# astaka-pe/Dual-DMP

Measured on AMD Instinct MI355X. Metric: training iters/sec + MAD score, 1M-face mesh @ 1/2/4/8 MI355X, higher is better.
Workload: dtype f32 (f16x3 split-MFMA GEMMs, f32 accumulate); 1 GPU; synthetic torus-grid manifold mesh, 1000000 faces / 500000 verts, float32 features, k=(3,4,4,4,1), bnfloop=1, native numbering (BASELINE.json configs[2]); faces=1000000, verts=500000, parallelism=1 GPU, hipgraph_replay=True, two_streams=True

## Files before the change

### dual-dmp_amd/csrc/gemm.hip

```cpp
#include "ddmp_common.h"
#include "finalize.h"
#include "gemm_tn_rm.h"

#include <algorithm>
#include <cstdlib>
#include <type_traits>
#include <vector>

namespace {

using namespace ddmp;

typedef float f32x16 __attribute__((ext_vector_type(16)));

constexpr int kBM = 128;
constexpr int kBK = 32;
constexpr int kLd = kBK + 4;

template <int TN, bool B_KMAJOR, bool PRO>
__global__ __launch_bounds__(256) void gemm_rows_kernel(
    const float* __restrict__ A, int64_t lda, const float* __restrict__ B, int64_t ldb,
    float* __restrict__ Y, int64_t ldy, int n_rows, int KD, int MD,
    const float* __restrict__ bias, const float* __restrict__ pscale, const float* __restrict__ pshift,
    float slope, int n_row_tiles, int n_col_tiles) {
// ... 471 lines not shown
                            int64_t n_rows) {
    return panel_enabled() && n_rows >= panel_min_rows(KD, MD) && KD % 32 == 0 && KD >= 32 && (KD >= 64 || MD <= 128) &&
           MD % 4 == 0 && MD >= 16 && MD <= 512 && ws &&
           (reinterpret_cast<uintptr_t>(ws) & 15) == 0 && ws_bytes >= ddmp_gemm_rows_workspace_bytes(KD, MD) &&
           ldy >= MD && Y;
}
static bool rr_enabled() {
    static int e = -1;
    if (e < 0) {
        const char* v = getenv("DDMP_GEMM_RR");
        e = (v && atoi(v) == 0) ? 0 : 1;
    }
    return e == 1;
}
static inline bool rr_route_ok(int64_t n_rows, int KD, int64_t lda, int64_t lda2) {
    return rr_enabled() && KD >= 64 && KD <= 512 && n_rows >= kRRMinRows &&
           n_rows * lda * 4 < ((int64_t)1 << 32) && n_rows * lda2 * 4 < ((int64_t)1 << 32);
}
template <int PM>
static void f16s_measure(const float* A, int64_t lda, const float* A2, int64_t lda2, int64_t n_rows, int C,
                         const float* pa, const float* pb, const float* pk1, const float* pk0, float slope, float* slot,
                         hipStream_t st) {
    (void)hipMemsetAsync(slot, 0, 16, st);
    const int64_t total = n_rows * (C / 4);
    const int grid = (int)std::min<int64_t>(cdiv(total, 256 * 8), 8 * device_cus());
    hipLaunchKernelGGL((f16s_absmax_kernel<PM>), dim3((unsigned)std::max(grid, 1)), dim3(256), 0, st, A, lda, A2, lda2,
                       n_rows, C, pa, pb, pk1, pk0, slope, slot);
}

template <int PM>
static void launch_panel(int mode, const float* A, int64_t lda, const float* A2, int64_t lda2, const float* W,
                         int64_t ldw, int transpose, void* planes, float* Y, int64_t ldy, int n_rows, int KD, int MD,
                         const float* bias, const float* ps, const float* psh, const float* pc1, const float* pc0,
                         float slope, hipStream_t st, double* stats, double* sums, ddmp::CallCtx& ctx,
                         const float* red_yp = nullptr, int64_t red_ldyp = 0,
                         const float* const* red_bn4 = nullptr ) {
    const int WC = MD > 256 ? 4 : MD > 128 ? 2 : 1, WR = 8 / WC;
    const int NJ = MD > 128 ? 4 : MD > 64 ? 4 : MD > 32 ? 2 : 1;
    const int MP = 32 * NJ * WC, BMR = 64 * WR;
    const int n_row_tiles = (int)ddmp::cdiv(n_rows, BMR);
    const int64_t total = (int64_t)MP * KD;
    const int sgrid = (int)std::min<int64_t>(ddmp::cdiv(total, 256), 1024);
    dim3 grid((unsigned)std::min(n_row_tiles, device_cus())), block(512);
    const int f16 = (mode == 6 && WC > 1 && lda % 4 == 0 && (PM != 2 || lda2 % 4 == 0)) ? gemm_f16() : 0;
    if (f16) {
        char* tail = (char*)planes + (size_t)2 * MP * KD * 2;
        float* wscale = (float*)tail;
        float* slot = ctx.slot_a ? ctx.slot_a : (float*)(tail + 16);
        const bool prime = !ctx.slot_a || ctx.prime;
        const bool w_ready = w_prepared(ctx.prepared, W, ldw, planes, kWPanelF16, 2, MD, KD, transpose, MP);
        if (!w_ready) {
            (void)hipMemsetAsync(wscale, 0, 4, st);
            hipLaunchKernelGGL(f16s_wmax_kernel, dim3((unsigned)std::min(transpose ? KD : MD, 128)), dim3(256), 0, st, W, ldw,
                               transpose ? KD : MD, transpose ? MD : KD, wscale);
        }
        const bool rr = rr_route_ok(n_rows, KD, lda, PM == 2 ? lda2 : 0) && !(PM == 2 && MD > kRRCols);
        if (!w_ready)
            hipLaunchKernelGGL((split_w_panel_kernel<2, _Float16>), dim3(sgrid), dim3(256), 0, st, W, ldw, MD, KD, transpose, MP,
                               (_Float16*)planes, (const float*)wscale);
        if (prime) f16s_measure<PM>(A, lda, A2, lda2, n_rows, KD, ps, psh, pc1, pc0, slope, slot, st);
        const int target = prime ? kF16TargetExact : kF16TargetStale;
        const void* Bh = planes;
        if (rr) {
            const int n_halves = MP / kRRCols;
            const int tiles = (int)ddmp::cdiv(n_rows, kRRRows);
            const int slots = std::max(8, std::min((tiles + 7) / 8 * 8, 2 * device_cus() / n_halves / 8 * 8));
            dim3 rgrid((unsigned)(slots * n_halves)), rblock(256);
            for (int heal = 0; heal <= (prime ? 0 : 1); ++heal) {
                if (PM == 0 && stats && red_yp)
                    hipLaunchKernelGGL((gemm_rr_kernel<0, 2, 3>), rgrid, rblock, 0, st, A, lda, A2, lda2, (const _Float16*)Bh, MP,
                                       Y, ldy, n_rows, KD, MD, bias, ps, psh, pc1, pc0, slope, tiles, stats, slot,
                                       (const float*)wscale, target, heal, red_yp, red_ldyp, red_bn4[0], red_bn4[1], red_bn4[2],
                                       red_bn4[3]);
                else if (PM != 2 && stats)
                    hipLaunchKernelGGL((gemm_rr_kernel<PM == 2 ? 0 : PM, 1, 3>), rgrid, rblock, 0, st, A, lda, A2, lda2,
                                       (const _Float16*)Bh, MP, Y, ldy, n_rows, KD, MD, bias, ps, psh, pc1, pc0, slope, tiles,
                                       stats, slot, (const float*)wscale, target, heal);
                else
                    hipLaunchKernelGGL((gemm_rr_kernel<PM, 0, PM == 2 ? 2 : 3>), rgrid, rblock, 0, st, A, lda, A2, lda2, (const _Float16*)Bh, MP,
                                       Y, ldy, n_rows, KD, MD, bias, ps, psh, pc1, pc0, slope, tiles, stats, slot,
                                       (const float*)wscale, target, heal);
            }
            if (stats && sums) {
                const size_t pbytes = ((size_t)tiles * 2 * 2 * MP * sizeof(double) + 255) / 256 * 256;
                fpartials_reduce(stats, tiles * 2, MP, MD, (double*)((char*)stats + pbytes), sums, st, ctx.take_fin(MD));
            }
            return;
        }
#define DDMP_PANEL_H(WR_, WC_, AR_, HEAL_)                                                                        \
    hipLaunchKernelGGL((gemm_panel_kernel<WR_, WC_, AR_, PM, 4>), grid, block, 0, st, A, lda, A2, lda2, Bh, Y, ldy,   \
                       n_rows, KD, MD, bias, ps, psh, pc1, pc0, slope, n_row_tiles, stats, slot, (const float*)wscale, \
                       target, HEAL_)
        for (int heal = 0; heal <= (prime ? 0 : 1); ++heal) {
            if (WC == 4) {
                DDMP_PANEL_H(2, 4, 13, heal);
            } else {
                DDMP_PANEL_H(4, 2, 13, heal);
            }
        }
#undef DDMP_PANEL_H
        if (stats && sums) {
            const size_t pbytes = ((size_t)n_row_tiles * WR * 2 * MP * sizeof(double) + 255) / 256 * 256;
            fpartials_reduce(stats, n_row_tiles * WR, MP, MD, (double*)((char*)stats + pbytes), sums, st, ctx.take_fin(MD));
        }
        return;
    }
    if (w_prepared(ctx.prepared, W, ldw, planes, kWPanelB16, mode == 6 ? 3 : 2, MD, KD, transpose, MP)) {
    } else if (mode == 6)
        hipLaunchKernelGGL((split_w_panel_kernel<3, __bf16>), dim3(sgrid), dim3(256), 0, st, W, ldw, MD, KD, transpose, MP, (__bf16*)planes, (const float*)nullptr);
    else
        hipLaunchKernelGGL((split_w_panel_kernel<2, __bf16>), dim3(sgrid), dim3(256), 0, st, W, ldw, MD, KD, transpose, MP, (__bf16*)planes, (const float*)nullptr);
    const void* Bp = planes;
#define DDMP_PANEL(WR_, WC_, NT_, NJ_)                                                                            \
    hipLaunchKernelGGL((gemm_panel_kernel<WR_, WC_, NT_, PM, NJ_>), grid, block, 0, st, A, lda, A2, lda2, Bp, Y, ldy, \
                       n_rows, KD, MD, bias, ps, psh, pc1, pc0, slope, n_row_tiles, stats, (float*)nullptr,            \
                       (const float*)nullptr, 0, 0)
    if (WC == 1 && PM == 0 && stats && red_yp && (NJ == 4 || NJ == 2)) {
#define DDMP_PANEL_RS(NT_, NJ_)                                                                                     \
    hipLaunchKernelGGL((gemm_panel_kernel<8, 1, NT_, 0, NJ_, true>), grid, block, 0, st, A, lda, A2, lda2, Bp, Y, ldy, \
                       n_rows, KD, MD, bias, ps, psh, pc1, pc0, slope, n_row_tiles, stats, (float*)nullptr,            \
                       (const float*)nullptr, 0, 0, red_yp, red_ldyp, red_bn4[0], red_bn4[1], red_bn4[2], red_bn4[3])
        if constexpr (PM == 0) {
            if (NJ == 4) {
                if (mode == 6) DDMP_PANEL_RS(3, 4); else DDMP_PANEL_RS(2, 4);
            } else {
                if (mode == 6) DDMP_PANEL_RS(3, 2); else DDMP_PANEL_RS(2, 2);
            }
        }
#undef DDMP_PANEL_RS
    } else if (WC == 4) {
        if (mode == 6) DDMP_PANEL(2, 4, 3, 4); else DDMP_PANEL(2, 4, 2, 4);
    } else if (WC == 2) {
        if (mode == 6) DDMP_PANEL(4, 2, 3, 4); else DDMP_PANEL(4, 2, 2, 4);
    } else {
        if (NJ == 4) {
            if (mode == 6) DDMP_PANEL(8, 1, 3, 4); else DDMP_PANEL(8, 1, 2, 4);
        } else if (NJ == 2) {
            if (mode == 6) DDMP_PANEL(8, 1, 3, 2); else DDMP_PANEL(8, 1, 2, 2);
        } else {
            if (mode == 6) DDMP_PANEL(8, 1, 3, 1); else DDMP_PANEL(8, 1, 2, 1);
        }
    }
#undef DDMP_PANEL
    if (stats && sums) {
        const size_t pbytes = ((size_t)n_row_tiles * WR * 2 * MP * sizeof(double) + 255) / 256 * 256;
        fpartials_reduce(stats, n_row_tiles * WR, MP, MD, (double*)((char*)stats + pbytes), sums, st, ctx.take_fin(MD));
    }
}

static inline bool ws_ok(int KD, int MD, const float* Y, int64_t ldy, const void* ws, size_t ws_bytes) {
    return ws_enabled() && KD % 32 == 0 && KD >= 96 && MD % 4 == 0 && MD <= 1024 && ldy % 4 == 0 &&
           (reinterpret_cast<uintptr_t>(Y) & 15) == 0 && ws && (reinterpret_cast<uintptr_t>(ws) & 15) == 0 &&
           ws_bytes >= ddmp_gemm_rows_workspace_bytes(KD, MD);
}

static int g_gemm_mode = -1, g_gemm_f16 = 0;
static int gemm_mode() {
    if (g_gemm_mode < 0) {
        const char* e = getenv("DDMP_GEMM_MODE");
        int m = e ? atoi(e) : 13;
        g_gemm_f16 = m == 13 ? m : 0;
        g_gemm_mode = (m == 0 || m == 3 || m == 6) ? m : 6;
    }
    return g_gemm_mode;
}
static int gemm_f16() {
    (void)gemm_mode();
    return g_gemm_f16;
}
extern "C" int ddmp_set_gemm_mode(int mode) {
    if (mode != 0 && mode != 3 && mode != 6 && mode != 13) return DDMP_EINVAL;
    g_gemm_f16 = mode > 10 ? mode : 0;
    g_gemm_mode = mode > 10 ? 6 : mode;
    return DDMP_OK;
}
extern "C" int ddmp_get_gemm_mode(void) { return gemm_f16() ? gemm_f16() : gemm_mode(); }

extern "C" int ddmp_gemm_scales_roll(float* slots, int n_slots, ddmp_stream stream) {
    ARG_TRY(slots && n_slots > 0);
    hipLaunchKernelGGL(f16s_roll_kernel, dim3((unsigned)cdiv(n_slots, 64)), dim3(64), 0, (hipStream_t)stream, slots, n_slots);
    LAUNCH_TRY();
    return DDMP_OK;
}

static inline bool aligned16(const void* p) { return (reinterpret_cast<uintptr_t>(p) & 15) == 0; }

extern "C" size_t ddmp_gemm_rows_workspace_bytes(int K, int M) {
    if (K <= 0 || M <= 0) return 0;
    const size_t kp = ((size_t)K + 127) / 128 * 128, mp = ((size_t)M + 127) / 128 * 128;
    return 3 * kp * mp * 2;
}

static bool presplit_w(const float* W, int64_t ldw, int M, int K, int transpose, void* ws, size_t ws_bytes,
                       hipStream_t st, bool prepared) {
    const int mode = gemm_mode();
    const int RK = transpose ? M : K;
    if (mode == 0 || !ws || ws_bytes < ddmp_gemm_rows_workspace_bytes(K, M) || RK % 8 != 0 ||
        (reinterpret_cast<uintptr_t>(ws) & 15))
        return false;
    const int grid = (int)std::min<int64_t>(cdiv((int64_t)M * K, 256), 1024);
    if (w_prepared(prepared, W, ldw, ws, kWPlain, mode == 6 ? 3 : 2, M, K, transpose, 0)) return true;
    if (mode == 6)
        hipLaunchKernelGGL((split_w_kernel<3>), dim3(grid), dim3(256), 0, st, W, ldw, M, K, transpose, (__bf16*)ws);
    else
        hipLaunchKernelGGL((split_w_kernel<2>), dim3(grid), dim3(256), 0, st, W, ldw, M, K, transpose, (__bf16*)ws);
    return hipGetLastError() == hipSuccess;
}

static WPrepDesc plan_w(int form, int64_t n_rows, const float* W, int64_t ldw, int M, int K, int has_pro, void* planes,
                        size_t planes_bytes) {
    WPrepDesc d{W, planes, ldw, 0, 0, 0, 0, 0, 0};
    const int mode = gemm_mode();
    if (mode == 0 || !planes || (reinterpret_cast<uintptr_t>(planes) & 15) || planes_bytes < ddmp_gemm_rows_workspace_bytes(K, M))
        return d;
    const int KD = form ? M : K, MD = form ? K : M;
    d.transpose = form ? 1 : 0;
    d.nterm = mode == 6 ? 3 : 2;
    float dummy;
    if (!(has_pro && KD > 512) && panel_ok(KD, MD, &dummy, MD, planes, planes_bytes, n_rows)) {
        const int WC = MD > 256 ? 4 : MD > 128 ? 2 : 1;
        const int NJ = MD > 128 ? 4 : MD > 64 ? 4 : MD > 32 ? 2 : 1;
        d.P = 32 * NJ * WC;
        d.MD = MD;
        d.KD = KD;
        if (mode == 6 && WC > 1 && gemm_f16()) {
            d.kind = kWPanelF16;
            d.nterm = 2;
        } else {
            d.kind = kWPanelB16;
// ... 479 lines not shown
```

### dual-dmp_amd/csrc/gemm_panel.inc

```

constexpr int kPanelThreads = 512;

__device__ __forceinline__ int panel_sw(int r, int h) { return r * 16 + ((h ^ ((r >> 3) & 1)) << 3); }

template <int ARITH> struct Arith {
    static constexpr bool F16 = ARITH > 10;
    static constexpr int NTERM = ARITH == 3 ? 3 : 2;
    static constexpr int NP = ARITH == 3 ? 6 : ARITH == 14 ? 4 : 3;
    typedef typename std::conditional<F16, _Float16, __bf16>::type E;
    static constexpr int pa(int q) { return ARITH == 3 ? (q == 0 ? 0 : q == 1 ? 1 : q == 2 ? 2 : q == 3 ? 0 : q == 4 ? 1 : 0)
                                                       : (q == 0 ? 0 : q == 1 ? 1 : NP == 4 && q == 2 ? 1 : 0); }
    static constexpr int pb(int q) { return ARITH == 3 ? (q == 0 ? 2 : q == 1 ? 1 : q == 2 ? 0 : q == 3 ? 1 : 0)
                                                       : (q == 0 ? 1 : q == 1 ? 0 : NP == 4 && q == 2 ? 1 : 0); }
};

#include "gemm_f16s.inc"

template <int NTERM, typename E>
__device__ __forceinline__ void split_w_panel_body(const float* __restrict__ W, int64_t ldw, int MD, int KD, int transpose,
                                                   int MP, E* __restrict__ planes, float ws, int bid, int nblk) {
    const int ns = KD / kSK;
    const int total = ns * MP * kSK;
    for (int idx = bid * 256 + threadIdx.x; idx < total; idx += nblk * 256) {
        const int kk = idx % kSK;
        const int r = (idx / kSK) % MP;
        const int st = idx / (kSK * MP);
        const int c = st * kSK + kk;
        float x = 0.f;
        if (r < MD) x = (transpose ? W[(int64_t)c * ldw + r] : W[(int64_t)r * ldw + c]) * ws;
        E t[NTERM];
        split1<NTERM>(x, t);
        const int64_t base = (int64_t)st * NTERM * MP * kSK + panel_sw(r, kk >> 3) + (kk & 7);
#pragma unroll
        for (int q = 0; q < NTERM; ++q) planes[base + (int64_t)q * MP * kSK] = t[q];
    }
}
template <int NTERM, typename E>
__global__ __launch_bounds__(256) void split_w_panel_kernel(const float* __restrict__ W, int64_t ldw, int MD, int KD,
                                                            int transpose, int MP, E* __restrict__ planes,
                                                            const float* __restrict__ wscale) {
    split_w_panel_body<NTERM, E>(W, ldw, MD, KD, transpose, MP, planes, wscale ? f16s_wscale(wscale) : 1.f, blockIdx.x,
                                 gridDim.x);
}

__device__ __forceinline__ void panel_barrier_lds() {
    __builtin_amdgcn_sched_barrier(0);
    asm volatile("s_waitcnt lgkmcnt(0)\n\ts_barrier" ::: "memory");
    __builtin_amdgcn_sched_barrier(0);
}

__device__ __forceinline__ float4 f4_bn_bwd(float4 dz, float4 y, float4 a, float4 b, float4 k1, float4 k0, float g1, float gs) {
    float4 o;
    o.x = fmaf(a.x, dz.x * (fmaf(y.x, a.x, b.x) > 0.f ? g1 : gs), fmaf(k1.x, y.x, k0.x));
    o.y = fmaf(a.y, dz.y * (fmaf(y.y, a.y, b.y) > 0.f ? g1 : gs), fmaf(k1.y, y.y, k0.y));
    o.z = fmaf(a.z, dz.z * (fmaf(y.z, a.z, b.z) > 0.f ? g1 : gs), fmaf(k1.z, y.z, k0.z));
    o.w = fmaf(a.w, dz.w * (fmaf(y.w, a.w, b.w) > 0.f ? g1 : gs), fmaf(k1.w, y.w, k0.w));
    return o;
}

__device__ __forceinline__ void panel_barrier(int vm_outstanding) {
    __builtin_amdgcn_sched_barrier(0);
    if (vm_outstanding == 1) asm volatile("s_waitcnt vmcnt(1) lgkmcnt(0)\n\ts_barrier" ::: "memory");
    else if (vm_outstanding == 2) asm volatile("s_waitcnt vmcnt(2) lgkmcnt(0)\n\ts_barrier" ::: "memory");
    else if (vm_outstanding == 4) asm volatile("s_waitcnt vmcnt(4) lgkmcnt(0)\n\ts_barrier" ::: "memory");
    else if (vm_outstanding == 5) asm volatile("s_waitcnt vmcnt(5) lgkmcnt(0)\n\ts_barrier" ::: "memory");
    else if (vm_outstanding == 6) asm volatile("s_waitcnt vmcnt(6) lgkmcnt(0)\n\ts_barrier" ::: "memory");
    else if (vm_outstanding == 8) asm volatile("s_waitcnt vmcnt(8) lgkmcnt(0)\n\ts_barrier" ::: "memory");
    else asm volatile("s_waitcnt vmcnt(0) lgkmcnt(0)\n\ts_barrier" ::: "memory");
    __builtin_amdgcn_sched_barrier(0);
}

#include "fpartials.inc"


template <int WR, int WC, int ARITH, int PM, int NJ = 4, bool RS = false>
__global__ __launch_bounds__(512) void gemm_panel_kernel(
    const float* __restrict__ A, int64_t lda, const float* __restrict__ A2, int64_t lda2,
    const void* __restrict__ Bp_ , float* __restrict__ Y, int64_t ldy, int n_rows, int KD, int MD,
    const float* __restrict__ bias, const float* __restrict__ pscale, const float* __restrict__ pshift,
    const float* __restrict__ pc1, const float* __restrict__ pc0, float slope, int n_row_tiles,
    double* __restrict__ stats ,
    float* __restrict__ aslot , const float* __restrict__ wscale ,
    int target, int heal ,
    const float* __restrict__ rs_yp = nullptr, int64_t rs_ldyp = 0, const float* __restrict__ rs_scale = nullptr,
    const float* __restrict__ rs_shift = nullptr, const float* __restrict__ rs_mean = nullptr,
    const float* __restrict__ rs_rstd = nullptr) {
    typedef Arith<ARITH> AR;
    typedef typename AR::E E;
    typedef typename V16<E>::v8 E8;
    constexpr int NTERM = AR::NTERM, NP = AR::NP;
    constexpr bool F16 = AR::F16;
    const E* __restrict__ Bp = static_cast<const E*>(Bp_);
    constexpr bool PRO = PM != 0;
    static_assert(WR * WC == 8, "eight waves");
    constexpr int BMR = 64 * WR, WN = 32 * NJ, MP = WN * WC;
    constexpr int NA = WR / 2;
    constexpr int NL = PM == 2 ? 2 * NA : NA;
    constexpr int kAStage = NTERM * BMR * kSK, kBStage = NTERM * MP * kSK;
    constexpr int NCH = kBStage * 2 / 1024;
    constexpr int NB = F16 ? 3 : 2;
    constexpr int kProF = (PM == 2 ? 4 : PM == 1 ? 2 : 0) * kMaxProK;
    __shared__ __attribute__((aligned(16))) unsigned char smem[NB * (kAStage + kBStage) * 2 + 512 * 4 + kProF * 4 + (RS ? 4 * 512 * 4 : 0) + 16];
    E* As = reinterpret_cast<E*>(smem);
    E* Bs = As + NB * kAStage;
    float* s_bias = reinterpret_cast<float*>(Bs + NB * kBStage);
    float* s_pro = s_bias + 512;
    float* s_red = s_pro + kProF;

    const int tid = threadIdx.x, lane = tid & 63;
    const int wave = __builtin_amdgcn_readfirstlane(tid >> 6);
    const int wr = wave / WC, wc = wave % WC;
    const int l31 = lane & 31, lh = lane >> 5;
    const int ns = KD / kSK;
    const int my_tiles = (n_row_tiles - (int)blockIdx.x + (int)gridDim.x - 1) / (int)gridDim.x;
    const int G = my_tiles * ns;
    const int last_t = (int)blockIdx.x + (my_tiles - 1) * (int)gridDim.x;
    float sa = 1.f, out_scale = 1.f, amax = 0.f;
    if (F16) {
        float in_use = aslot[0];
        if (heal) {
            if (reinterpret_cast<const unsigned*>(aslot)[2] == 0u) return;
            in_use = aslot[1];
            target = kF16TargetExact;
        }
        sa = f16s_scale(in_use, target);
        out_scale = (1.f / sa) * (1.f / f16s_wscale(wscale));
    }

    const float fs = F16 ? sa : 1.f, fss = fs * slope;
    if (PRO) {
        for (int i = tid; i < KD; i += 512) {
            s_pro[i] = PM == 1 ? pscale[i] * fs : pscale[i];
            s_pro[kMaxProK + i] = PM == 1 ? pshift[i] * fs : pshift[i];
            if (PM == 2) {
                s_pro[2 * kMaxProK + i] = pc1[i] * fs;
                s_pro[3 * kMaxProK + i] = pc0[i] * fs;
            }
        }
    }
    for (int i = tid; i < MP; i += 512) s_bias[i] = (bias && i < MD) ? bias[i] : 0.f;
    if (RS) {
        for (int i = tid; i < MP; i += 512) {
            const bool con = i < MD;
            s_red[i] = con ? rs_scale[i] : 0.f;
            s_red[512 + i] = con ? rs_shift[i] : 0.f;
            s_red[1024 + i] = con ? rs_mean[i] : 0.f;
            s_red[1536 + i] = con ? rs_rstd[i] : 0.f;
        }
    }
    __syncthreads();

    const int kq = tid & 3, ar = tid >> 2;
    struct Ring {
        float4 a[NA];
        float4 a2[PM == 2 ? NA : 1];
    };
    Ring R[NB];
    const float* aptr[NA];
    const float* a2ptr[NA];
    int lt = blockIdx.x, lk = 0;
    auto a_tile = [&](int t) {
#pragma unroll
        for (int p = 0; p < NA; ++p) {
            const int64_t row = min(t * BMR + p * 128 + ar, n_rows - 1);
            aptr[p] = A + row * lda + kq * 4;
            if (PM == 2) a2ptr[p] = A2 + row * lda2 + kq * 4;
        }
    };
    a_tile(lt);
    auto a_load = [&](Ring& r) {
#pragma unroll
        for (int p = 0; p < NA; ++p) {
            r.a[p] = *reinterpret_cast<const float4*>(aptr[p] + lk);
            if (PM == 2) r.a2[p] = *reinterpret_cast<const float4*>(a2ptr[p] + lk);
        }
    };
    auto a_advance = [&]() {
        lk += kSK;
        if (lk == KD) {
            lk = 0;
            lt = min(lt + (int)gridDim.x, last_t);
            a_tile(lt);
        }
    };
    int sk = 0;
    auto a_store = [&](int buf, const Ring& r, int p) {
        float4 v = r.a[p];
        if (PM == 1) {
            const float4 sc = *reinterpret_cast<const float4*>(&s_pro[sk + kq * 4]);
            const float4 sh = *reinterpret_cast<const float4*>(&s_pro[kMaxProK + sk + kq * 4]);
// ... 33 lines not shown
        ++bk;
        const bool wrap = bk == ns;
        bk = wrap ? 0 : bk;
        bsrc = wrap ? Bp + lane * 8 : bsrc + kBStage;
    };

    f32x16 acc[2][NJ];
    auto zero_acc = [&]() {
#pragma unroll
        for (int i = 0; i < 2; ++i)
#pragma unroll
            for (int j = 0; j < NJ; ++j)
#pragma unroll
                for (int r = 0; r < 16; ++r) acc[i][j][r] = 0.f;
    };
    const int a_off = panel_sw(wr * 64 + l31, lh);
    const int b_off = panel_sw(wc * WN + l31, lh);
    E8 af[2][NTERM], bf[NJ][NTERM];
    auto rd = [&](int buf, int t) {
        const E* as = As + buf * kAStage + a_off;
        const E* bs = Bs + buf * kBStage + b_off;
#pragma unroll
        for (int i = 0; i < 2; ++i)
            af[i][AR::pa(t)] = *reinterpret_cast<const E8*>(as + AR::pa(t) * (BMR * kSK) + i * 512);
#pragma unroll
        for (int j = 0; j < NJ; ++j)
            bf[j][AR::pb(t)] = *reinterpret_cast<const E8*>(bs + AR::pb(t) * (MP * kSK) + j * 512);
    };
    auto mm = [&](int q) {
#pragma unroll
        for (int i = 0; i < 2; ++i)
#pragma unroll
            for (int j = 0; j < NJ; ++j)
                acc[i][j] = mfma16(af[i][AR::pa(q)], bf[j][AR::pb(q)], acc[i][j]);
    };
#define DDMP_FENCE_() __builtin_amdgcn_sched_barrier(0)
#define DDMP_PHASE_(N_DSR, N_VALU_PER, N_DSW, VMEM_PER) DDMP_PHASE_N_(8, N_DSR, N_VALU_PER, N_DSW, VMEM_PER)
#define DDMP_PHASE_N_(NM, N_DSR, N_VALU_PER, N_DSW, VMEM_PER)                               \
    _Pragma("unroll") for (int q_ = 0; q_ < (NM); ++q_) {                                   \
        __builtin_amdgcn_sched_group_barrier(0x008, 1, 0);                                  \
        if (q_ < (N_DSR)) __builtin_amdgcn_sched_group_barrier(0x100, 1, 0);                \
        if ((N_VALU_PER) > 0) __builtin_amdgcn_sched_group_barrier(0x002, (N_VALU_PER), 0); \
        if (q_ >= (NM) - (N_DSW)) __builtin_amdgcn_sched_group_barrier(0x200, 1, 0);        \
        if ((VMEM_PER) > 0) __builtin_amdgcn_sched_group_barrier(0x020, (VMEM_PER), 0);     \
    }
#ifdef DDMP_PANEL_ABLATE
#define DDMP_AB_(bit, stmt) do { if (!((DDMP_PANEL_ABLATE) & (bit))) { stmt; } } while (0)
#else
#define DDMP_AB_(bit, stmt) do { stmt; } while (0)
#endif
    auto iteration = [&](int buf, int bufa, int bufw, Ring& rl, const Ring& rs) {
        constexpr int NM = 2 * NJ;
        constexpr int NF = 2 + NJ;
        DDMP_AB_(16, rd(buf, 0));
        DDMP_FENCE_();
        DDMP_AB_(1, mm(0));
        DDMP_AB_(16, rd(buf, 1));
#pragma unroll
        for (int p = 0; p < (NA + 1) / 2; ++p) DDMP_AB_(2, a_store(bufa, rs, p));
        DDMP_PHASE_N_(NM, NF, (NA > 2 ? 12 : 6) * 8 / NM, NM < NTERM ? NM : NTERM, 0)
        DDMP_FENCE_();
        DDMP_AB_(1, mm(1));
        if (NTERM == 3) DDMP_AB_(16, rd(buf, 2));
#pragma unroll
        for (int p = (NA + 1) / 2; p < NA; ++p) DDMP_AB_(2, a_store(bufa, rs, p));
        a_store_done();
        DDMP_PHASE_N_(NM, NTERM == 3 ? NF : 0, NA >= 2 ? (NA > 2 ? 12 : 6) * 8 / NM : 0, NA >= 2 ? (NM < NTERM ? NM : NTERM) : 0, 0)
        DDMP_FENCE_();
        DDMP_AB_(1, mm(2));
        DDMP_AB_(4, b_copy(bufw));
        asm volatile("" ::: "memory");
        DDMP_AB_(8, a_load(rl));
        DDMP_PHASE_N_(NM, 0, 1, 0, NM >= 8 ? 1 : 2)
        DDMP_FENCE_();
        if (NP > 3) DDMP_AB_(1, mm(3));
        if (NP > 4) {
            DDMP_AB_(1, mm(4));
            DDMP_AB_(1, mm(5));
        }
    };
    auto epilogue = [&](int t) {
        const int row_base = t * BMR + wr * 64 + 4 * lh;
        const bool full = (t + 1) * BMR <= n_rows && MD == MP;
#pragma unroll
        for (int j = 0; j < NJ; ++j) {
            const int col = wc * WN + j * 32 + l31;
            const float bv = s_bias[col];
            float* yp = Y + (int64_t)row_base * ldy + col;
            if (PM != 2 && full) {
#pragma unroll
                for (int i = 0; i < 2; ++i)
#pragma unroll
                    for (int r = 0; r < 16; ++r) {
                        const int ro = i * 32 + (r & 3) + 8 * (r >> 2);
                        acc[i][j][r] = F16 ? fmaf(acc[i][j][r], out_scale, bv) : acc[i][j][r] + bv;
#if defined(DDMP_PANEL_ABLATE) && ((DDMP_PANEL_ABLATE) & 32)
                        if (acc[i][j][r] == 123.456f)
#endif
                        yp[(int64_t)ro * ldy] = acc[i][j][r];
                    }
            } else {
#pragma unroll
                for (int i = 0; i < 2; ++i)
#pragma unroll
                    for (int r = 0; r < 16; ++r) {
                        const int ro = i * 32 + (r & 3) + 8 * (r >> 2);
                        acc[i][j][r] = F16 ? fmaf(acc[i][j][r], out_scale, bv) : acc[i][j][r] + bv;
                        if (row_base + ro < n_rows && col < MD) yp[(int64_t)ro * ldy] = acc[i][j][r];
                    }
            }
            if (RS) {
                const float sc = s_red[col], sh = s_red[512 + col];
                const float mu = s_red[1024 + col], rs = s_red[1536 + col];
                const float* yq = rs_yp + (int64_t)row_base * rs_ldyp + col;
                float af = 0.f, bf = 0.f;
#pragma unroll
                for (int i = 0; i < 2; ++i)
#pragma unroll
                    for (int r = 0; r < 16; ++r) {
                        const int ro = i * 32 + (r & 3) + 8 * (r >> 2);
                        const bool ok = (full || (row_base + ro < n_rows && col < MD));
                        const float y = ok ? yq[(int64_t)ro * rs_ldyp] : 0.f;
                        const float g = ok ? acc[i][j][r] * lrelu_grad(fmaf(y, sc, sh), slope) : 0.f;
                        af += g;
                        bf = fmaf(g, (y - mu) * rs, bf);
                    }
                double s1 = (double)af, s2 = (double)bf;
                s1 += __shfl_xor(s1, 32, 64);
                s2 += __shfl_xor(s2, 32, 64);
                if (lh == 0) {
                    double* sp = stats + ((int64_t)(t * WR + wr) * 2) * MP + col;
                    sp[0] = s1;
                    sp[MP] = s2;
                }
            } else if (stats) {
                double s1 = 0.0, s2 = 0.0;
#pragma unroll
                for (int i = 0; i < 2; ++i)
#pragma unroll
                    for (int r = 0; r < 16; ++r) {
                        const int ro = i * 32 + (r & 3) + 8 * (r >> 2);
                        const double v = (full || row_base + ro < n_rows) ? (double)acc[i][j][r] : 0.0;
                        s1 += v;
                        s2 = fma(v, v, s2);
                    }
                s1 += __shfl_xor(s1, 32, 64);
                s2 += __shfl_xor(s2, 32, 64);
                if (lh == 0) {
                    double* sp = stats + ((int64_t)(t * WR + wr) * 2) * MP + col;
                    sp[0] = s1;
                    sp[MP] = s2;
                }
            }
        }
    };

    zero_acc();
    int cur_t = blockIdx.x, cnt = 0;
    auto stage_done = [&]() {
        if (++cnt == ns) {
            cnt = 0;
            epilogue(cur_t);
            zero_acc();
            cur_t += gridDim.x;
        }
    };
    if constexpr (NB == 2) {
        b_copy(0);
        a_load(R[0]);
        a_advance();
        a_load(R[1]);
        a_advance();
#pragma unroll
        for (int p = 0; p < NA; ++p) a_store(0, R[0], p);
        a_store_done();
        panel_barrier(NL);
        for (int g = 0; g < G; g += 2) {
            iteration(0, 1, 1, R[0], R[1]);
            a_advance();
            stage_done();
            panel_barrier(NL);
            iteration(1, 0, 0, R[1], R[0]);
            a_advance();
            stage_done();
            panel_barrier(NL);
        }
    } else {
        constexpr int NV = NCH / 8 + NL;
        static_assert(NCH % 8 == 0, "each wave issues the same number of W copies");
        b_copy(0);
        b_copy(1);
        a_load(R[0]);
        a_advance();
        a_load(R[1]);
        a_advance();
        a_load(R[2]);
        a_advance();
#pragma unroll
        for (int p = 0; p < NA; ++p) a_store(0, R[0], p);
        a_store_done();
        panel_barrier(0);
        for (int g = 0; g < G; g += 3) {
            iteration(0, 1, 2, R[0], R[1]);
            a_advance();
            stage_done();
            panel_barrier(NV);
            if (g + 1 < G) {
                iteration(1, 2, 0, R[1], R[2]);
                a_advance();
                stage_done();
            }
            panel_barrier(NV);
            if (g + 2 < G) {
                iteration(2, 0, 1, R[2], R[0]);
                a_advance();
                stage_done();
            }
            panel_barrier(NV);
        }
        asm volatile("s_waitcnt vmcnt(0)" ::: "memory");
    }
    if (F16 && !heal) f16s_publish(aslot, amax * (1.f / sa), sa);
}

template <int ARITH, bool PRO, bool GDUAL>
__global__ __launch_bounds__(512) void gemm_tn_panel_kernel(
    const float* __restrict__ G, int64_t ldg, const float* __restrict__ G2, int64_t ldg2,
    const float* __restrict__ Z, int64_t ldz, float* __restrict__ out,
    int64_t ld_out, int64_t split_stride, int n_rows, int M, int K, int rows_per_split, int n_tiles_m,
    int n_tiles_k, int n_splits, const float* __restrict__ pscale, const float* __restrict__ pshift,
    const float* __restrict__ ga, const float* __restrict__ gb, const float* __restrict__ gk1,
    const float* __restrict__ gk0, float slope, float* __restrict__ gslot, float* __restrict__ zslot, int target,
    int heal) {
    typedef Arith<ARITH> AR;
    typedef typename AR::E E;
    typedef typename V16<E>::v8 E8;
    constexpr int NTERM = AR::NTERM, NP = AR::NP;
    constexpr bool F16 = AR::F16;
    constexpr int BT = 256;
    constexpr int kPlane = BT * kSK;
    __shared__ __attribute__((aligned(16))) E Gs[2][NTERM][kPlane];
    __shared__ __attribute__((aligned(16))) E Zs[2][NTERM][kPlane];

    const int n_tiles = n_tiles_m * n_tiles_k;
    const int xcd = blockIdx.x & (kXcd - 1), local = blockIdx.x >> 3;
    const int tile = local % n_tiles;
    const int split = (local / n_tiles) * kXcd + xcd;
    if (split >= n_splits) return;
    const int tm0 = (tile / n_tiles_k) * BT, tk0 = (tile % n_tiles_k) * BT;
    const int r_begin = split * rows_per_split;
    const int r_end = min(n_rows, r_begin + rows_per_split);

    const int tid = threadIdx.x, lane = tid & 63;
    const int wave = __builtin_amdgcn_readfirstlane(tid >> 6);
    const int wr = wave >> 1, wc = wave & 1;
    const int l31 = lane & 31, lh = lane >> 5;
    const int c = tid & (BT - 1), g = tid >> 8;
    const int gc = tm0 + c, zc = tk0 + c;
    const float* gcolp = G + min(gc, M - 1);
    const float* zcolp = Z + min(zc, K - 1);
    float sc = 1.f, sh = 0.f;
    if (PRO && zc < K) {
        sc = pscale[zc];
        sh = pshift[zc];
    }
    float ba = 0.f, bb = 0.f, bk1 = 0.f, bk0 = 0.f;
    const float* g2colp = G2 + min(gc, M - 1);
    if (GDUAL && gc < M) {
        ba = ga[gc];
        bb = gb[gc];
        bk1 = gk1[gc];
        bk0 = gk0[gc];
    }
    float sg = 1.f, sz = 1.f, gmax = 0.f, zmax = 0.f;
    if (F16) {
        float g_use = gslot[0], z_use = zslot[0];
        if (heal) {
            if ((reinterpret_cast<const unsigned*>(gslot)[2] | reinterpret_cast<const unsigned*>(zslot)[2]) == 0u) return;
            g_use = gslot[1];
            z_use = zslot[1];
            target = kF16TargetExact;
        }
        sg = f16s_scale(g_use, target);
        sz = f16s_scale(z_use, target);
    }
    constexpr int NS = NP == 3 ? 2 : 1;
    float rg[NS][8], rz[NS][8], rg2[NS][GDUAL ? 8 : 1];
    int grow = r_begin + g * 8;
    const float* gp = gcolp + (int64_t)grow * ldg;
    const float* g2p = g2colp + (int64_t)grow * ldg2;
    const float* zp = zcolp + (int64_t)grow * ldz;
    int zrow = grow;
    auto load_g = [&](int sl, int) {
        if (grow + 8 <= n_rows) {
#pragma unroll
            for (int e = 0; e < 8; ++e) {
                rg[sl][e] = gp[(int64_t)e * ldg];
                if (GDUAL) rg2[sl][GDUAL ? e : 0] = g2p[(int64_t)e * ldg2];
            }
        } else {
#pragma unroll
            for (int e = 0; e < 8; ++e) {
                const int64_t back = (int64_t)(grow + e) - min(grow + e, n_rows - 1);
// ... 145 lines not shown
```

### dual-dmp_amd/csrc/gemm_rr.inc

```

constexpr int kRRCols = 256;
constexpr int kRRRows = 128;
constexpr int kRRStage = 2 * kRRCols * kSK;
constexpr int kRRASlot = 32 * kSK;

__device__ __forceinline__ void rr_dma16(unsigned voff, const void* sbase, unsigned lds_dst_uniform) {
    unsigned keep;
    asm volatile("s_mov_b32 %0, m0\n\ts_mov_b32 m0, %3\n\ts_nop 0\n\tglobal_load_lds_dwordx4 %1, %2\n\ts_mov_b32 m0, %0"
                 : "=&s"(keep)
                 : "v"(voff), "s"(sbase), "s"(lds_dst_uniform)
                 : "memory");
}
template <int N>
__device__ __forceinline__ void rr_wait() {
    __builtin_amdgcn_sched_barrier(0);
    asm volatile("s_waitcnt vmcnt(%0)" ::"n"(N) : "memory");
    __builtin_amdgcn_sched_barrier(0);
}
template <int N>
__device__ __forceinline__ void rr_wait_barrier() {
    __builtin_amdgcn_sched_barrier(0);
    asm volatile("s_waitcnt vmcnt(%0) lgkmcnt(0)\n\ts_barrier" ::"n"(N) : "memory");
    __builtin_amdgcn_sched_barrier(0);
}
// ... 143 lines not shown
            const float sh[8] = {sh0.x, sh0.y, sh0.z, sh0.w, sh1.x, sh1.y, sh1.z, sh1.w};
            if (PM == 1) {
#pragma unroll
                for (int e = 0; e < 8; ++e) v[e] = lrelu(fmaf(v[e], sc[e], sh[e]), slope);
            } else {
                const float* as2 = as + kARing;
                const float4 y0 = *reinterpret_cast<const float4*>(as2 + a_rd), y1 = *reinterpret_cast<const float4*>(as2 + (a_rd ^ 4));
                const float4 ka = *reinterpret_cast<const float4*>(cp + 2 * kMaxProK), kb = *reinterpret_cast<const float4*>(cp + 2 * kMaxProK + 4);
                const float4 la = *reinterpret_cast<const float4*>(cp + 3 * kMaxProK), lb = *reinterpret_cast<const float4*>(cp + 3 * kMaxProK + 4);
                const float k1[8] = {ka.x, ka.y, ka.z, ka.w, kb.x, kb.y, kb.z, kb.w};
                const float k0[8] = {la.x, la.y, la.z, la.w, lb.x, lb.y, lb.z, lb.w};
                const float y[8] = {y0.x, y0.y, y0.z, y0.w, y1.x, y1.y, y1.z, y1.w};
#pragma unroll
                for (int e = 0; e < 8; ++e)
                    v[e] = fmaf(sc[e], v[e] * (fmaf(y[e], sc[e], sh[e]) > 0.f ? sa : sas), fmaf(k1[e], y[e], k0[e]));
            }
        }
        typedef unsigned u32x4 __attribute__((ext_vector_type(4)));
        u32x4 ph, pm;
#pragma unroll
        for (int e = 0; e < 8; e += 4) {
            float4 x;
            x.x = PM ? v[e] : v[e] * sa;
            x.y = PM ? v[e + 1] : v[e + 1] * sa;
            x.z = PM ? v[e + 2] : v[e + 2] * sa;
            x.w = PM ? v[e + 3] : v[e + 3] * sa;
            amax = fmaxf(fmaxf(amax, fabsf(x.x)), fmaxf(fabsf(x.y), fmaxf(fabsf(x.z), fabsf(x.w))));
            uint2 h, m;
            f16_split_quad(x, h, m);
            ph[e >> 1] = h.x; ph[(e >> 1) + 1] = h.y;
            pm[e >> 1] = m.x; pm[(e >> 1) + 1] = m.y;
        }
        h1 = __builtin_bit_cast(E8, ph);
        h2 = __builtin_bit_cast(E8, pm);
    };

    f32x16 acc[NJ];
    auto zero_acc = [&]() {
#pragma unroll
        for (int j = 0; j < NJ; ++j)
#pragma unroll
            for (int r = 0; r < 16; ++r) acc[j][r] = 0.f;
    };
    const int b_off = panel_sw(l31, lh);
    auto kstep = [&](int cslot, const E8& a1, const E8& a2) {
        const E* bs = Bs + cslot * kRRStage + b_off;
        E8 b1[2], b2[2];
#pragma unroll
        for (int u = 0; u < 2; ++u) b2[u] = *reinterpret_cast<const E8*>(bs + kRRCols * kSK + u * 512);
#pragma unroll
        for (int u = 0; u < 2; ++u) b1[u] = *reinterpret_cast<const E8*>(bs + u * 512);
        __builtin_amdgcn_sched_group_barrier(0x100, 4, 0);
#pragma unroll
        for (int j = 0; j < NJ; j += 2) {
            constexpr bool kReload = !(DDMP_RR_ABLATE & 1);
            const bool reload = j + 2 < NJ && (kReload || (j & 2));
            acc[j] = mfma16(a1, b2[0], acc[j]);
            acc[j + 1] = mfma16(a1, b2[1], acc[j + 1]);
            if (reload) {
#pragma unroll
                for (int u = 0; u < 2; ++u) b2[u] = *reinterpret_cast<const E8*>(bs + kRRCols * kSK + (j + 2 + u) * 512);
            }
            if (!(DDMP_RR_ABLATE & 4)) {
                acc[j] = mfma16(a2, b1[0], acc[j]);
                acc[j + 1] = mfma16(a2, b1[1], acc[j + 1]);
            }
            acc[j] = mfma16(a1, b1[0], acc[j]);
            acc[j + 1] = mfma16(a1, b1[1], acc[j + 1]);
            if (reload) {
#pragma unroll
                for (int u = 0; u < 2; ++u) b1[u] = *reinterpret_cast<const E8*>(bs + (j + 2 + u) * 512);
            }
        }
#if DDMP_RR_ABLATE == 0
#pragma unroll
        for (int j = 0; j < NJ; j += 2) {
            __builtin_amdgcn_sched_group_barrier(0x008, 2, 0);
            if (j + 2 < NJ) __builtin_amdgcn_sched_group_barrier(0x100, 2, 0);
            __builtin_amdgcn_sched_group_barrier(0x008, 4, 0);
            if (j + 2 < NJ) __builtin_amdgcn_sched_group_barrier(0x100, 2, 0);
        }
#endif
    };
    auto epilogue = [&](int t, int free_slot) {
        const int row_base = t * kRRRows + wave * 32 + 4 * lh;
        const bool full = (t + 1) * kRRRows <= n_rows && col0 + kRRCols <= MD;
#pragma unroll
        for (int j = 0; j < NJ; ++j) {
            const int col = col0 + j * 32 + l31;
            const float bv = s_bias[j * 32 + l31];
            float* yp = Y + (int64_t)row_base * ldy + col;
            if (full) {
#pragma unroll
                for (int r = 0; r < 16; ++r) {
                    const int ro = (r & 3) + 8 * (r >> 2);
                    acc[j][r] = fmaf(acc[j][r], out_scale, bv);
                    yp[(int64_t)ro * ldy] = acc[j][r];
                }
            } else {
#pragma unroll
                for (int r = 0; r < 16; ++r) {
                    const int ro = (r & 3) + 8 * (r >> 2);
                    acc[j][r] = fmaf(acc[j][r], out_scale, bv);
                    if (row_base + ro < n_rows && col < MD) yp[(int64_t)ro * ldy] = acc[j][r];
                }
            }
        }
        if (STATS) {
            const int g = wave >> 1, o = wave & 1;
            double* xch = reinterpret_cast<double*>(Bs + free_slot * kRRStage);
            auto colsum = [&](int j, double& a, double& b) {
                a = 0.0;
                b = 0.0;
                if (STATS == 1) {
#pragma unroll
                    for (int r = 0; r < 16; ++r) {
                        const int ro = (r & 3) + 8 * (r >> 2);
                        const double v = (full || row_base + ro < n_rows) ? (double)acc[j][r] : 0.0;
                        a += v;
                        b = fma(v, v, b);
                    }
                } else {
                    const int col = col0 + j * 32 + l31;
                    const float sc = s_red[j * 32 + l31], sh = s_red[kRRCols + j * 32 + l31];
                    const float mu = s_red[2 * kRRCols + j * 32 + l31], rs = s_red[3 * kRRCols + j * 32 + l31];
                    const float* yq = Yp + (int64_t)row_base * ldyp + col;
                    float y[16];
                    if (full) {
#pragma unroll
                        for (int r = 0; r < 16; ++r) y[r] = yq[(int64_t)((r & 3) + 8 * (r >> 2)) * ldyp];
                    } else {
#pragma unroll
                        for (int r = 0; r < 16; ++r) {
                            const int ro = (r & 3) + 8 * (r >> 2);
                            y[r] = (col < MD && row_base + ro < n_rows) ? yq[(int64_t)ro * ldyp] : 0.f;
                        }
                    }
                    float af = 0.f, bf = 0.f;
#pragma unroll
                    for (int r = 0; r < 16; ++r) {
                        const int ro = (r & 3) + 8 * (r >> 2);
                        const float g = (full || row_base + ro < n_rows) ? acc[j][r] * lrelu_grad(fmaf(y[r], sc, sh), slope) : 0.f;
                        af += g;
                        bf = fmaf(g, (y[r] - mu) * rs, bf);
                    }
                    a = (double)af;
                    b = (double)bf;
                }
                a += __shfl_xor(a, 32, 64);
                b += __shfl_xor(b, 32, 64);
            };
            double* give = xch + (g * 2 + o) * 256;
            const double* take = xch + (g * 2 + (o ^ 1)) * 256;
            double* sp = stats + ((int64_t)(t * 2 + g) * 2) * MPW + col0;
            auto give_tiles = [&](auto role) {
                constexpr int O = decltype(role)::value;
#pragma unroll
                for (int jj = 0; jj < NJ / 2; ++jj) {
                    double a, b;
                    colsum(O ? jj + NJ / 2 : jj, a, b);
                    if (lh == 0) {
                        give[jj * 32 + l31] = a;
                        give[128 + jj * 32 + l31] = b;
                    }
                    __builtin_amdgcn_sched_barrier(0);
                }
            };
            auto keep_tiles = [&](auto role) {
                constexpr int O = decltype(role)::value;
#pragma unroll
                for (int jj = 0; jj < NJ / 2; ++jj) {
                    const int j = O ? jj : jj + NJ / 2;
                    double a, b;
                    colsum(j, a, b);
                    if (lh == 0) {
                        sp[j * 32 + l31] = a + take[jj * 32 + l31];
                        sp[MPW + j * 32 + l31] = b + take[128 + jj * 32 + l31];
                    }
                    __builtin_amdgcn_sched_barrier(0);
                }
            };
            if (o) give_tiles(std::integral_constant<int, 1>()); else give_tiles(std::integral_constant<int, 0>());
            rr_lds_barrier();
            if (o) keep_tiles(std::integral_constant<int, 1>()); else keep_tiles(std::integral_constant<int, 0>());
            rr_lds_barrier();
        }
    };

    zero_acc();
#pragma unroll
    for (int i = 0; i < NB - 1; ++i) issue();
    static_assert(NB == 2 || NB == 3, "ring depth");
    rr_wait_barrier<NA + (NB - 2) * NV>();
    int cur_t = slot, cslot = 0, kt = 0;
    for (int g = 0; g < G; ++g) {
        issue();
        rr_wait<(NB - 1) * NV>();
        E8 a1, a2;
        convert(cslot, kt, a1, a2);
        __builtin_amdgcn_sched_barrier(0);
        kstep(cslot, a1, a2);
        rr_wait_barrier<NA + (NB - 2) * NV>();
        const int done = cslot;
        cslot = cslot + 1 == NB ? 0 : cslot + 1;
        if (++kt == ns) {
            kt = 0;
            epilogue(cur_t, done);
            zero_acc();
            cur_t += n_slots;
        }
    }
    asm volatile("s_waitcnt vmcnt(0)" ::: "memory");
    if (!heal) f16s_publish(aslot, amax * (1.f / sa), sa);
}
```

Before: 23.27 iters/s.

## Accumulate GEMM column-stat partials per block before writing to global

Persistent GEMM kernels (panel and rr variants) now accumulate per-tile column sum/sumsq partials in registers or LDS across all tiles a block processes. Each block writes a single record at the end instead of one record per row tile. The host-side reduction then sums only grid-size records rather than tiles×WR records. This cuts global partial-stat traffic and the size of the final reduction, at the cost of extra LDS, a trailing block-wide barrier and reduction, and reliance on each block's first tile equalling blockIdx.x.

```diff
diff --git a/dual-dmp_amd/csrc/gemm.hip b/dual-dmp_amd/csrc/gemm.hip
--- a/dual-dmp_amd/csrc/gemm.hip
+++ b/dual-dmp_amd/csrc/gemm.hip
@@ -577,8 +577,9 @@
                                        (const float*)wscale, target, heal);
             }
             if (stats && sums) {
-                const size_t pbytes = ((size_t)tiles * 2 * 2 * MP * sizeof(double) + 255) / 256 * 256;
-                fpartials_reduce(stats, tiles * 2, MP, MD, (double*)((char*)stats + pbytes), sums, st, ctx.take_fin(MD));
+                const int records = std::min(slots, tiles);
+                const size_t pbytes = ((size_t)records * 2 * MP * sizeof(double) + 255) / 256 * 256;
+                fpartials_reduce(stats, records, MP, MD, (double*)((char*)stats + pbytes), sums, st, ctx.take_fin(MD));
             }
             return;
         }
@@ -595,8 +596,8 @@
         }
 #undef DDMP_PANEL_H
         if (stats && sums) {
-            const size_t pbytes = ((size_t)n_row_tiles * WR * 2 * MP * sizeof(double) + 255) / 256 * 256;
-            fpartials_reduce(stats, n_row_tiles * WR, MP, MD, (double*)((char*)stats + pbytes), sums, st, ctx.take_fin(MD));
+            const size_t pbytes = ((size_t)grid.x * 2 * MP * sizeof(double) + 255) / 256 * 256;
+            fpartials_reduce(stats, (int)grid.x, MP, MD, (double*)((char*)stats + pbytes), sums, st, ctx.take_fin(MD));
         }
         return;
     }
@@ -638,8 +639,8 @@
     }
 #undef DDMP_PANEL
     if (stats && sums) {
-        const size_t pbytes = ((size_t)n_row_tiles * WR * 2 * MP * sizeof(double) + 255) / 256 * 256;
-        fpartials_reduce(stats, n_row_tiles * WR, MP, MD, (double*)((char*)stats + pbytes), sums, st, ctx.take_fin(MD));
+        const size_t pbytes = ((size_t)grid.x * 2 * MP * sizeof(double) + 255) / 256 * 256;
+        fpartials_reduce(stats, (int)grid.x, MP, MD, (double*)((char*)stats + pbytes), sums, st, ctx.take_fin(MD));
     }
 }
 
diff --git a/dual-dmp_amd/csrc/gemm_panel.inc b/dual-dmp_amd/csrc/gemm_panel.inc
--- a/dual-dmp_amd/csrc/gemm_panel.inc
+++ b/dual-dmp_amd/csrc/gemm_panel.inc
@@ -100,12 +100,15 @@
     constexpr int NCH = kBStage * 2 / 1024;
     constexpr int NB = F16 ? 3 : 2;
     constexpr int kProF = (PM == 2 ? 4 : PM == 1 ? 2 : 0) * kMaxProK;
-    __shared__ __attribute__((aligned(16))) unsigned char smem[NB * (kAStage + kBStage) * 2 + 512 * 4 + kProF * 4 + (RS ? 4 * 512 * 4 : 0) + 16];
+    constexpr bool kSt = RS || PM != 2;
+    constexpr int kRunD = kSt ? WR * 2 * MP : 0;
+    __shared__ __attribute__((aligned(16))) unsigned char smem[NB * (kAStage + kBStage) * 2 + 512 * 4 + kProF * 4 + (RS ? 4 * 512 * 4 : 0) + kRunD * 8 + 16];
     E* As = reinterpret_cast<E*>(smem);
     E* Bs = As + NB * kAStage;
     float* s_bias = reinterpret_cast<float*>(Bs + NB * kBStage);
     float* s_pro = s_bias + 512;
     float* s_red = s_pro + kProF;
+    double* s_run = reinterpret_cast<double*>(s_red + (RS ? 4 * 512 : 0));
 
     const int tid = threadIdx.x, lane = tid & 63;
     const int wave = __builtin_amdgcn_readfirstlane(tid >> 6);
@@ -305,6 +308,7 @@
     auto epilogue = [&](int t) {
         const int row_base = t * BMR + wr * 64 + 4 * lh;
         const bool full = (t + 1) * BMR <= n_rows && MD == MP;
+        const bool first = t == (int)blockIdx.x;
 #pragma unroll
         for (int j = 0; j < NJ; ++j) {
             const int col = wc * WN + j * 32 + l31;
@@ -352,11 +356,11 @@
                 s1 += __shfl_xor(s1, 32, 64);
                 s2 += __shfl_xor(s2, 32, 64);
                 if (lh == 0) {
-                    double* sp = stats + ((int64_t)(t * WR + wr) * 2) * MP + col;
-                    sp[0] = s1;
-                    sp[MP] = s2;
+                    double* sp = s_run + (wr * 2) * MP + col;
+                    sp[0] = (first ? 0.0 : sp[0]) + s1;
+                    sp[MP] = (first ? 0.0 : sp[MP]) + s2;
                 }
-            } else if (stats) {
+            } else if (kSt && stats) {
                 double s1 = 0.0, s2 = 0.0;
 #pragma unroll
                 for (int i = 0; i < 2; ++i)
@@ -370,9 +374,9 @@
                 s1 += __shfl_xor(s1, 32, 64);
                 s2 += __shfl_xor(s2, 32, 64);
                 if (lh == 0) {
-                    double* sp = stats + ((int64_t)(t * WR + wr) * 2) * MP + col;
-                    sp[0] = s1;
-                    sp[MP] = s2;
+                    double* sp = s_run + (wr * 2) * MP + col;
+                    sp[0] = (first ? 0.0 : sp[0]) + s1;
+                    sp[MP] = (first ? 0.0 : sp[MP]) + s2;
                 }
             }
         }
@@ -442,6 +446,15 @@
             panel_barrier(NV);
         }
         asm volatile("s_waitcnt vmcnt(0)" ::: "memory");
+    }
+    if (kSt && (RS || stats)) {
+        __syncthreads();
+        for (int i = tid; i < 2 * MP; i += 512) {
+            double s = 0.0;
+#pragma unroll
+            for (int w = 0; w < WR; ++w) s += s_run[w * 2 * MP + i];
+            stats[(int64_t)blockIdx.x * 2 * MP + i] = s;
+        }
     }
     if (F16 && !heal) f16s_publish(aslot, amax * (1.f / sa), sa);
 }
diff --git a/dual-dmp_amd/csrc/gemm_rr.inc b/dual-dmp_amd/csrc/gemm_rr.inc
--- a/dual-dmp_amd/csrc/gemm_rr.inc
+++ b/dual-dmp_amd/csrc/gemm_rr.inc
@@ -249,6 +249,9 @@
         }
 #endif
     };
+    double run[STATS ? NJ / 2 : 1][2];
+#pragma unroll
+    for (int jj = 0; jj < (STATS ? NJ / 2 : 1); ++jj) run[jj][0] = run[jj][1] = 0.0;
     auto epilogue = [&](int t, int free_slot) {
         const int row_base = t * kRRRows + wave * 32 + 4 * lh;
         const bool full = (t + 1) * kRRRows <= n_rows && col0 + kRRCols <= MD;
@@ -319,7 +322,6 @@
             };
             double* give = xch + (g * 2 + o) * 256;
             const double* take = xch + (g * 2 + (o ^ 1)) * 256;
-            double* sp = stats + ((int64_t)(t * 2 + g) * 2) * MPW + col0;
             auto give_tiles = [&](auto role) {
                 constexpr int O = decltype(role)::value;
 #pragma unroll
@@ -340,10 +342,8 @@
                     const int j = O ? jj : jj + NJ / 2;
                     double a, b;
                     colsum(j, a, b);
-                    if (lh == 0) {
-                        sp[j * 32 + l31] = a + take[jj * 32 + l31];
-                        sp[MPW + j * 32 + l31] = b + take[128 + jj * 32 + l31];
-                    }
+                    run[jj][0] += a + take[jj * 32 + l31];
+                    run[jj][1] += b + take[128 + jj * 32 + l31];
                     __builtin_amdgcn_sched_barrier(0);
                 }
             };
@@ -378,5 +378,26 @@
         }
     }
     asm volatile("s_waitcnt vmcnt(0)" ::: "memory");
+    if (STATS) {
+        const int g = wave >> 1, o = wave & 1;
+        double* mine = reinterpret_cast<double*>(As + wave * (NB * kRRASlot));
+        const double* upper = reinterpret_cast<const double*>(As + (wave + 2) * (NB * kRRASlot));
+        if (g == 1 && lh == 0) {
+#pragma unroll
+            for (int jj = 0; jj < NJ / 2; ++jj) {
+                mine[jj * 32 + l31] = run[jj][0];
+                mine[128 + jj * 32 + l31] = run[jj][1];
+            }
+        }
+        rr_lds_barrier();
+        if (g == 0 && lh == 0) {
+            double* sp = stats + ((int64_t)slot * 2) * MPW + col0 + (o ? 0 : NJ / 2) * 32;
+#pragma unroll
+            for (int jj = 0; jj < NJ / 2; ++jj) {
+                sp[jj * 32 + l31] = run[jj][0] + upper[jj * 32 + l31];
+                sp[MPW + jj * 32 + l31] = run[jj][1] + upper[128 + jj * 32 + l31];
+            }
+        }
+    }
     if (!heal) f16s_publish(aslot, amax * (1.f / sa), sa);
 }
```

Measured after the change: 23.37 iters/s, median of 6. Within noise of the previous version (+0.4%).
